# kkromberg/SpeechRecognition

Hardware: AMD Instinct MI355X
Metric: frames/sec scored+decoded (higher is better)
Workload: dtype f64

## Files before the change

speechrecognition_amd/csrc/gmm_prefilter.hip:

```cpp
#include <hip/hip_runtime.h>
#include <stdint.h>

#include <algorithm>
#include <cmath>
#include <vector>

#include "kernels.h"

#ifndef SR_P16_NB
#define SR_P16_NB 4
#endif

namespace srgpu {

typedef float v4f __attribute__((ext_vector_type(4)));
static constexpr int kPWaves = 4;
static constexpr int kGroupBlocks = 8;

typedef _Float16 f16x8 __attribute__((ext_vector_type(8)));

__device__ inline uint32_t pack_f16x2(_Float16 l, _Float16 h) {
  return (uint32_t)__builtin_bit_cast(uint16_t, l) | ((uint32_t)__builtin_bit_cast(uint16_t, h) << 16);
}

template <int KS32, int NB>
__global__ __launch_bounds__(kPWaves * 64, (NB <= 2 ? 3 : 2)) void gmm_prefilter16_kernel(GmmPrefilterArgs a) {
  constexpr int kBlockBytes = KS32 * 1024;
  constexpr int kStageBytes = kGroupBlocks * kBlockBytes;
  constexpr int kChunksPerStage = kStageBytes / 1024;
  constexpr int kDmaPerWave = kChunksPerStage / kPWaves;
  static_assert(kChunksPerStage % kPWaves == 0, "every wave issues the same number of LDS-DMA pieces per stage");
  constexpr int kTileFrames = kPWaves * NB * 16;
  constexpr size_t kTileBytes = (size_t)kTileFrames * (16 * KS32) * sizeof(float);
  constexpr size_t kLdsBytes = 2 * kStageBytes > kTileBytes ? 2 * kStageBytes : kTileBytes;
  __shared__ __attribute__((aligned(1024))) unsigned char lds[kLdsBytes];

  const int lane = threadIdx.x & 63, wave = threadIdx.x >> 6;
  const int g = lane >> 4, c = lane & 15;
  uint32_t x, y;
  {
    const uint32_t id = blockIdx.x;
    if ((a.ny & 7u) == 0) { const uint32_t j = id >> 3; y = (id & 7u) + 8u * (j / a.nx); x = j % a.nx; }
    else { y = id / a.nx; x = id % a.nx; }
  }
  const uint32_t g0 = a.split_begin[y], g1 = a.split_begin[y + 1];
  const uint64_t frame0 = (uint64_t)x * kTileFrames + (uint64_t)wave * (NB * 16);

  uint4 bf[NB][KS32];
  float bnorm[NB], dbnorm[NB];
  {
    float* fl = reinterpret_cast<float*>(lds);
    const uint64_t tile_first = (uint64_t)x * kTileFrames;
    const uint64_t tile_frames = (a.n_frames - tile_first < (uint64_t)kTileFrames) ? a.n_frames - tile_first : kTileFrames;
    const uint32_t n_floats = (uint32_t)tile_frames * a.dim;
    const float* src = a.feats + tile_first * a.dim;
    for (uint32_t i = threadIdx.x; i < n_floats; i += kPWaves * 64) fl[i] = src[i];
    __syncthreads();
#pragma unroll
    for (int nb = 0; nb < NB; nb++) {
      const uint32_t row = (uint32_t)wave * (NB * 16) + nb * 16 + c;
      const bool valid = row < tile_frames;
      const float* xr = fl + (valid ? row : 0u) * a.dim;
      float n2 = 0.0f, e2 = 0.0f;
#pragma unroll
      for (int ks = 0; ks < KS32; ks++) {
        _Float16 v[8];
#pragma unroll
        for (int j = 0; j < 8; j++) {
          const uint32_t k = 32u * ks + 8u * g + j, d = k >> 1;
          const float xf = (valid && d < a.dim) ? xr[d < a.dim ? d : 0u] : 0.0f;
          const float b = (k & 1u) ? xf : xf * xf;
          n2 += b * b;
          _Float16 h = (_Float16)b;
          const float bh = (float)h;
          const float e = (k & 1u) ? xf - bh : __builtin_fmaf(xf, xf, -bh);
          e2 += e * e;
          if (valid && k >= 2u * a.dim && k < 2u * a.dim + 3u) h = (_Float16)1.0f;
          v[j] = h;
        }
        bf[nb][ks] = make_uint4(pack_f16x2(v[0], v[1]), pack_f16x2(v[2], v[3]), pack_f16x2(v[4], v[5]), pack_f16x2(v[6], v[7]));
      }
      n2 += __shfl_xor(n2, 16);
      n2 += __shfl_xor(n2, 32);
      e2 += __shfl_xor(e2, 16);
      e2 += __shfl_xor(e2, 32);
      bnorm[nb] = sqrtf(n2) * 1.0001f;
      dbnorm[nb] = fminf(sqrtf(e2) * 1.0001f, kPfRes16 * bnorm[nb]);
    }
    __syncthreads();
  }

  const unsigned char* dma_src = a.apack + (uint64_t)g0 * kStageBytes + (uint64_t)wave * 1024 + lane * 16;
  auto issue_stage = [&](int buf) {
#pragma unroll
    for (int i = 0; i < kDmaPerWave; i++) {
      const int chunk = i * kPWaves + wave;
      unsigned char* dst = lds + buf * kStageBytes + chunk * 1024;
      __builtin_amdgcn_global_load_lds((const __attribute__((address_space(1))) void*)(dma_src + i * (kPWaves * 1024)),
                                       (__attribute__((address_space(3))) void*)dst, 16, 0, 0);
    }
    dma_src += kStageBytes;
  };
  auto frag = [&](int buf, int j, int ks) -> f16x8 {
    return __builtin_bit_cast(f16x8, *reinterpret_cast<const uint4*>(lds + buf * kStageBytes + j * kBlockBytes + ks * 1024 + lane * 16));
  };

  const uint32_t n_stages = g1 - g0;
  if (n_stages > 0) issue_stage(0);
  if (n_stages > 1) issue_stage(1);
  if (n_stages > 1) __builtin_amdgcn_s_waitcnt(0x0F70 | kDmaPerWave);
  else __builtin_amdgcn_s_waitcnt(0x0F70);
  __syncthreads();
  f16x8 a_c, a_n;
  if (n_stages > 0) a_c = frag(0, 0, 0);
  uint32_t* m_ptr = a.mask + (uint64_t)g0 * a.n_frames * 4u;
  uint32_t m_off[NB];
  bool m_ok[NB];
#pragma unroll
  for (int nb = 0; nb < NB; nb++) {
    const uint64_t f = frame0 + (uint64_t)nb * 16 + c;
    m_ok[nb] = f < a.n_frames;
    m_off[nb] = (uint32_t)f * 4u + (uint32_t)g;
  }
  for (uint32_t s = 0; s < n_stages; s++) {
    const uint32_t grp = g0 + s;
    const int buf = s & 1;
    v4f ap[NB][kGroupBlocks];
#pragma unroll
    for (int j = 0; j < kGroupBlocks; j++) {
      v4f acc[NB];
#pragma unroll
      for (int nb = 0; nb < NB; nb++) acc[nb] = (v4f){0.f, 0.f, 0.f, 0.f};
#pragma unroll
      for (int ks = 0; ks < KS32; ks++) {
        if (j == kGroupBlocks - 1 && ks == KS32 - 1) {
          if (s + 1 < n_stages) {
            __builtin_amdgcn_s_waitcnt(0x0070);
            __syncthreads();
            if (s + 2 < n_stages) issue_stage(buf);
            a_n = frag(buf ^ 1, 0, 0);
          }
        } else {
          a_n = frag(buf, (ks == KS32 - 1) ? j + 1 : j, (ks == KS32 - 1) ? 0 : ks + 1);
        }
        __builtin_amdgcn_sched_barrier(0);
#pragma unroll
        for (int nb = 0; nb < NB; nb++)
          acc[nb] = __builtin_amdgcn_mfma_f32_16x16x32_f16(a_c, __builtin_bit_cast(f16x8, bf[nb][ks]), acc[nb], 0, 0, 0);
        __builtin_amdgcn_sched_barrier(0);
        a_c = a_n;
      }
#pragma unroll
      for (int nb = 0; nb < NB; nb++) ap[nb][j] = acc[nb];
    }
    const float4 lim = reinterpret_cast<const float4*>(a.grp_lim)[4u * grp + g];
#pragma unroll
    for (int nb = 0; nb < NB; nb++) {
      float amin = __builtin_huge_valf();
#pragma unroll
      for (int j = 0; j < kGroupBlocks; j += 2)
        asm("v_min3_f32 %0, %0, %1, %2\n\tv_min3_f32 %0, %0, %3, %4\n\tv_min3_f32 %0, %0, %5, %6\n\tv_min3_f32 %0, %0, %7, %8"
            : "+v"(amin)
            : "v"(ap[nb][j][0]), "v"(ap[nb][j][1]), "v"(ap[nb][j][2]), "v"(ap[nb][j][3]), "v"(ap[nb][j + 1][0]),
              "v"(ap[nb][j + 1][1]), "v"(ap[nb][j + 1][2]), "v"(ap[nb][j + 1][3]));
      if (a.chunks >= 2) { const float o = __shfl_xor(amin, 16); asm("v_min_f32 %0, %0, %1" : "+v"(amin) : "v"(o)); }
      if (a.chunks >= 4) { const float o = __shfl_xor(amin, 32); asm("v_min_f32 %0, %0, %1" : "+v"(amin) : "v"(o)); }
      const float limit = amin + __builtin_fmaf(lim.y, dbnorm[nb], __builtin_fmaf(lim.x, bnorm[nb], lim.z));
      uint32_t mask = 0;
#pragma unroll
      for (int j = kGroupBlocks - 1; j >= 1; j -= 2)
        asm("v_cmp_ngt_f32 vcc, %2, %1\n\tv_addc_co_u32 %0, vcc, %0, %0, vcc\n\t"
            "v_cmp_ngt_f32 vcc, %3, %1\n\tv_addc_co_u32 %0, vcc, %0, %0, vcc\n\t"
            "v_cmp_ngt_f32 vcc, %4, %1\n\tv_addc_co_u32 %0, vcc, %0, %0, vcc\n\t"
            "v_cmp_ngt_f32 vcc, %5, %1\n\tv_addc_co_u32 %0, vcc, %0, %0, vcc\n\t"
            "v_cmp_ngt_f32 vcc, %6, %1\n\tv_addc_co_u32 %0, vcc, %0, %0, vcc\n\t"
            "v_cmp_ngt_f32 vcc, %7, %1\n\tv_addc_co_u32 %0, vcc, %0, %0, vcc\n\t"
            "v_cmp_ngt_f32 vcc, %8, %1\n\tv_addc_co_u32 %0, vcc, %0, %0, vcc\n\t"
            "v_cmp_ngt_f32 vcc, %9, %1\n\tv_addc_co_u32 %0, vcc, %0, %0, vcc"
            : "+v"(mask)
            : "v"(limit), "v"(ap[nb][j][3]), "v"(ap[nb][j][2]), "v"(ap[nb][j][1]), "v"(ap[nb][j][0]), "v"(ap[nb][j - 1][3]),
              "v"(ap[nb][j - 1][2]), "v"(ap[nb][j - 1][1]), "v"(ap[nb][j - 1][0])
            : "vcc");
      if (m_ok[nb]) m_ptr[m_off[nb]] = mask;
    }
    m_ptr += a.n_frames * 4u;
  }
}

#ifndef SR_PS_PIN
#define SR_PS_PIN 1
#endif
#if SR_PS_PIN
#define SR_PS_PIN_FETCH __builtin_amdgcn_sched_barrier(0)
#else
#define SR_PS_PIN_FETCH (void)0
#endif
static constexpr int kSNB = 2;
static constexpr int kSRangeFrames = 2048;

template <int KS32>
__global__ __launch_bounds__(kPWaves * 64) void gmm_prefilter_operands_kernel(const float* feats, uint64_t n_frames, uint32_t dim,
                                                                              uint64_t n_blocks, uint4* bfrag, float2* bnorm) {
  const int lane = threadIdx.x & 63, wave = threadIdx.x >> 6;
  const uint32_t g = lane >> 4, c = lane & 15;
  const uint64_t blk = (uint64_t)blockIdx.x * kPWaves + wave;
  if (blk >= n_blocks) return;
  const uint64_t f = blk * 16 + c;
  const bool valid = f < n_frames;
  const float* xr = feats + (valid ? f : 0u) * dim;
  float n2 = 0.0f, e2 = 0.0f;
#pragma unroll
  for (int ks = 0; ks < KS32; ks++) {
    _Float16 v[8];
#pragma unroll
    for (int j = 0; j < 8; j++) {
      const uint32_t k = 32u * ks + 8u * g + j, d = k >> 1;
      const float xf = (valid && d < dim) ? xr[d < dim ? d : 0u] : 0.0f;
      const float b = (k & 1u) ? xf : xf * xf;
      n2 += b * b;
      _Float16 h = (_Float16)b;
      const float bh = (float)h;
      const float e = (k & 1u) ? xf - bh : __builtin_fmaf(xf, xf, -bh);
      e2 += e * e;
      if (valid && k >= 2u * dim && k < 2u * dim + 3u) h = (_Float16)1.0f;
      v[j] = h;
    }
    bfrag[(blk * KS32 + ks) * 64 + lane] =
        make_uint4(pack_f16x2(v[0], v[1]), pack_f16x2(v[2], v[3]), pack_f16x2(v[4], v[5]), pack_f16x2(v[6], v[7]));
  }
  n2 += __shfl_xor(n2, 16);
  n2 += __shfl_xor(n2, 32);
  e2 += __shfl_xor(e2, 16);
  e2 += __shfl_xor(e2, 32);
  const float bn = sqrtf(n2) * 1.0001f;
  const float dbn = fminf(sqrtf(e2) * 1.0001f, kPfRes16 * bn);
  if (g == 0) bnorm[f] = make_float2(bn, dbn);
}

struct GmmStationaryPlan { uint32_t n_quads, n_ranges, range_frames, per_xcd; };

template <int KS32>
__global__ __launch_bounds__(kPWaves * 64, 2) void gmm_prefilter_stationary_kernel(GmmPrefilterArgs a, GmmStationaryPlan p) {
  constexpr int NB = kSNB;
  constexpr int kGroupBytes = kGroupBlocks * KS32 * 1024;
  const int lane = threadIdx.x & 63, wave = threadIdx.x >> 6;
  const int g = lane >> 4, c = lane & 15;
  const uint32_t item = (blockIdx.x & 7u) * p.per_xcd + (blockIdx.x >> 3);
  if ((blockIdx.x >> 3) >= p.per_xcd || item >= p.n_quads * p.n_ranges) return;
  const uint32_t grp = (item % p.n_quads) * kPWaves + wave;
  if (grp >= a.n_groups) return;
  const uint64_t f_begin = (uint64_t)(item / p.n_quads) * p.range_frames;
  if (f_begin >= a.n_frames) return;
  const uint64_t f_end = f_begin + p.range_frames < a.n_frames ? f_begin + p.range_frames : a.n_frames;
  const uint32_t n_steps = (uint32_t)((f_end - f_begin + 16 * NB - 1) / (16 * NB));

  f16x8 af[kGroupBlocks][KS32];
  {
    const uint4* src = reinterpret_cast<const uint4*>(a.apack + (uint64_t)grp * kGroupBytes) + lane;
#pragma unroll
    for (int j = 0; j < kGroupBlocks; j++)
#pragma unroll
      for (int ks = 0; ks < KS32; ks++) af[j][ks] = __builtin_bit_cast(f16x8, src[(j * KS32 + ks) * 64]);
  }
  const float4 lim = reinterpret_cast<const float4*>(a.grp_lim)[4u * grp + g];

  const uint4* b_src = a.bfrag + (f_begin / 16) * (KS32 * 64) + lane;
  const float2* n_src = a.bnorm + f_begin + c;
  uint32_t* m_ptr = a.mask + (uint64_t)grp * a.n_frames * 4u;
  uint4 bq[2][NB][KS32];
  float2 nq[2][NB];
  auto fetch = [&](int buf, uint32_t s) __attribute__((always_inline)) {
    const uint4* bs = b_src + (uint64_t)s * (NB * KS32 * 64);
#pragma unroll
    for (int nb = 0; nb < NB; nb++) {
#pragma unroll
      for (int ks = 0; ks < KS32; ks++) bq[buf][nb][ks] = bs[(nb * KS32 + ks) * 64];
      nq[buf][nb] = n_src[(uint64_t)s * (NB * 16) + nb * 16];
    }
  };
  auto step = [&](int buf, uint32_t s) __attribute__((always_inline)) {
    v4f ap[NB][kGroupBlocks];
#pragma unroll
    for (int nb = 0; nb < NB; nb++)
#pragma unroll
      for (int j = 0; j < kGroupBlocks; j++) ap[nb][j] = (v4f){0.f, 0.f, 0.f, 0.f};
#pragma unroll
    for (int ks = 0; ks < KS32; ks++)
#pragma unroll
      for (int j = 0; j < kGroupBlocks; j++)
#pragma unroll
        for (int nb = 0; nb < NB; nb++)
          ap[nb][j] = __builtin_amdgcn_mfma_f32_16x16x32_f16(af[j][ks], __builtin_bit_cast(f16x8, bq[buf][nb][ks]), ap[nb][j], 0, 0, 0);
    __builtin_amdgcn_sched_barrier(0);
    asm volatile("s_nop 7");
    __builtin_amdgcn_sched_barrier(0);
#pragma unroll
    for (int nb = 0; nb < NB; nb++) {
      float amin = __builtin_huge_valf();
#pragma unroll
      for (int j = 0; j < kGroupBlocks; j += 2)
        asm("v_min3_f32 %0, %0, %1, %2\n\tv_min3_f32 %0, %0, %3, %4\n\tv_min3_f32 %0, %0, %5, %6\n\tv_min3_f32 %0, %0, %7, %8"
            : "+v"(amin)
            : "v"(ap[nb][j][0]), "v"(ap[nb][j][1]), "v"(ap[nb][j][2]), "v"(ap[nb][j][3]), "v"(ap[nb][j + 1][0]),
              "v"(ap[nb][j + 1][1]), "v"(ap[nb][j + 1][2]), "v"(ap[nb][j + 1][3]));
      if (a.chunks >= 2) { const float o = __shfl_xor(amin, 16); asm("v_min_f32 %0, %0, %1" : "+v"(amin) : "v"(o)); }
      if (a.chunks >= 4) { const float o = __shfl_xor(amin, 32); asm("v_min_f32 %0, %0, %1" : "+v"(amin) : "v"(o)); }
      const float limit = amin + __builtin_fmaf(lim.y, nq[buf][nb].y, __builtin_fmaf(lim.x, nq[buf][nb].x, lim.z));
      uint32_t mask = 0;
#pragma unroll
      for (int j = kGroupBlocks - 1; j >= 1; j -= 2)
        asm("v_cmp_ngt_f32 vcc, %2, %1\n\tv_addc_co_u32 %0, vcc, %0, %0, vcc\n\t"
            "v_cmp_ngt_f32 vcc, %3, %1\n\tv_addc_co_u32 %0, vcc, %0, %0, vcc\n\t"
            "v_cmp_ngt_f32 vcc, %4, %1\n\tv_addc_co_u32 %0, vcc, %0, %0, vcc\n\t"
            "v_cmp_ngt_f32 vcc, %5, %1\n\tv_addc_co_u32 %0, vcc, %0, %0, vcc\n\t"
            "v_cmp_ngt_f32 vcc, %6, %1\n\tv_addc_co_u32 %0, vcc, %0, %0, vcc\n\t"
            "v_cmp_ngt_f32 vcc, %7, %1\n\tv_addc_co_u32 %0, vcc, %0, %0, vcc\n\t"
            "v_cmp_ngt_f32 vcc, %8, %1\n\tv_addc_co_u32 %0, vcc, %0, %0, vcc\n\t"
            "v_cmp_ngt_f32 vcc, %9, %1\n\tv_addc_co_u32 %0, vcc, %0, %0, vcc"
            : "+v"(mask)
            : "v"(limit), "v"(ap[nb][j][3]), "v"(ap[nb][j][2]), "v"(ap[nb][j][1]), "v"(ap[nb][j][0]), "v"(ap[nb][j - 1][3]),
              "v"(ap[nb][j - 1][2]), "v"(ap[nb][j - 1][1]), "v"(ap[nb][j - 1][0])
            : "vcc");
      const uint64_t f = f_begin + (uint64_t)s * (NB * 16) + nb * 16 + c;
      if (f < a.n_frames) m_ptr[(uint32_t)f * 4u + (uint32_t)g] = mask;
    }
  };
  fetch(0, 0);
  for (uint32_t s = 0; s < n_steps; s += 2) {
    fetch(1, s + 1 < n_steps ? s + 1 : n_steps - 1);
    SR_PS_PIN_FETCH;
    step(0, s);
    if (s + 1 >= n_steps) break;
    fetch(0, s + 2 < n_steps ? s + 2 : n_steps - 1);
    SR_PS_PIN_FETCH;
    step(1, s + 1);
  }
}

__global__ void fp16_denormal_probe_kernel(float* out) {
  const int lane = threadIdx.x;
  f16x8 a = {0, 0, 0, 0, 0, 0, 0, 0}, b = {0, 0, 0, 0, 0, 0, 0, 0};
  if (lane < 16) { a[0] = (_Float16)9.5367431640625e-7f; b[0] = (_Float16)1024.0f; }
  v4f acc = {0.f, 0.f, 0.f, 0.f};
  acc = __builtin_amdgcn_mfma_f32_16x16x32_f16(a, b, acc, 0, 0, 0);
  out[lane] = acc[0];
}

hipError_t probe_fp16_denormals(hipStream_t stream, bool* preserved) {
  float* d = nullptr;
  hipError_t e = hipMalloc(reinterpret_cast<void**>(&d), 64 * sizeof(float));
  if (e != hipSuccess) return e;
  hipLaunchKernelGGL(fp16_denormal_probe_kernel, dim3(1), dim3(64), 0, stream, d);
  float h[64];
  e = hipGetLastError();
  if (e == hipSuccess) e = hipStreamSynchronize(stream);
  if (e == hipSuccess) e = hipMemcpy(h, d, sizeof(h), hipMemcpyDeviceToHost);
  (void)hipFree(d);
  if (e != hipSuccess) return e;
  *preserved = true;
  for (int i = 0; i < 64; i++) *preserved = *preserved && h[i] == 9.765625e-4f;
  return hipSuccess;
}

template <int KS>
__global__ void fp16_accumulation_probe_kernel(const _Float16* A, const _Float16* B, float* out) {
  constexpr int K = 32 * KS;
  const int lane = threadIdx.x, r = lane & 15, q = lane >> 4;
  v4f acc = {0.f, 0.f, 0.f, 0.f};
#pragma unroll
  for (int ks = 0; ks < KS; ks++) {
    f16x8 a, b;
#pragma unroll
    for (int j = 0; j < 8; j++) {
      const int k = 32 * ks + 8 * q + j;
      a[j] = A[r * K + k];
      b[j] = B[k * 16 + r];
    }
    acc = __builtin_amdgcn_mfma_f32_16x16x32_f16(a, b, acc, 0, 0, 0);
  }
#pragma unroll
  for (int i = 0; i < 4; i++) out[(4 * q + i) * 16 + r] = acc[i];
}

hipError_t probe_fp16_accumulation(hipStream_t stream, int ks32, bool* ok, double* worst_ratio) {
  if (ks32 != 3 && ks32 != 4) return hipErrorInvalidValue;
  const int kCases = 8;
  const int K = 32 * ks32;
  const double allowed = ks32 == 3 ? 87.0 : 132.0;
  std::vector<_Float16> hA((size_t)kCases * 16 * K), hB((size_t)kCases * K * 16);
  uint64_t rng = 0x9E3779B97F4A7C15ull;
  auto next = [&]() { rng ^= rng << 13; rng ^= rng >> 7; rng ^= rng << 17; return rng; };
  for (int t = 0; t < kCases; t++) {
    _Float16* A = hA.data() + (size_t)t * 16 * K;
    _Float16* B = hB.data() + (size_t)t * K * 16;
    for (int k = 0; k < K; k++)
      for (int c = 0; c < 16; c++) B[k * 16 + c] = (_Float16)1.0f;
    for (int r = 0; r < 16; r++)
      for (int k = 0; k < K; k++) {
        float a = 0.f;
        const int fam = (t * 16 + r) & 3;
        if (fam == 0) a = k == (r * 5) % K ? 4096.0f : 0.75f;
        else if (fam == 1) a = k >= K - 2 ? 0.f : ((k & 1) ? -1.f : 1.f) * (1024.0f + (float)(((k >> 1) * 7 + r) % 64) * ((k & 1) ? 0.5f : 0.53125f));
        else if (fam == 2) a = 1.0009765625f;
        else { const uint64_t u = next(); a = ((u & 1) ? -1.f : 1.f) * (1.0f + (float)((u >> 8) & 1023) / 1024.0f) * (float)(1u << ((u >> 20) % 12)); }
        A[r * K + k] = (_Float16)a;
      }
    for (int k = 0; k < K; k++)
      for (int c = 0; c < 16; c++) {
        const uint64_t u = next();
        float b = 1.0f + (float)((u >> 5) % 1024) / 1024.0f;
        if ((c & 3) == 0) b = 1.0f;
        if ((c & 3) == 1) b = 1.0009765625f;
        B[k * 16 + c] = (_Float16)b;
      }
    for (int c = 0; c < 16; c++)
      for (int r = 0; r < 16; r++)
        if (((t * 16 + r) & 3) == 0) B[((r * 5) % K) * 16 + c] = (_Float16)2048.0f;
  }
  _Float16 *dA = nullptr, *dB = nullptr;
  float* dO = nullptr;
  hipError_t e;
  if ((e = hipMalloc(reinterpret_cast<void**>(&dA), hA.size() * 2)) != hipSuccess) return e;
  if ((e = hipMalloc(reinterpret_cast<void**>(&dB), hB.size() * 2)) != hipSuccess) { (void)hipFree(dA); return e; }
  if ((e = hipMalloc(reinterpret_cast<void**>(&dO), (size_t)kCases * 256 * 4)) != hipSuccess) { (void)hipFree(dA); (void)hipFree(dB); return e; }
  std::vector<float> got((size_t)kCases * 256);
  e = hipMemcpy(dA, hA.data(), hA.size() * 2, hipMemcpyHostToDevice);
  if (e == hipSuccess) e = hipMemcpy(dB, hB.data(), hB.size() * 2, hipMemcpyHostToDevice);
  for (int t = 0; t < kCases && e == hipSuccess; t++) {
    if (ks32 == 3) hipLaunchKernelGGL(fp16_accumulation_probe_kernel<3>, dim3(1), dim3(64), 0, stream, dA + (size_t)t * 16 * K, dB + (size_t)t * K * 16, dO + (size_t)t * 256);
    else hipLaunchKernelGGL(fp16_accumulation_probe_kernel<4>, dim3(1), dim3(64), 0, stream, dA + (size_t)t * 16 * K, dB + (size_t)t * K * 16, dO + (size_t)t * 256);
    e = hipGetLastError();
  }
  if (e == hipSuccess) e = hipStreamSynchronize(stream);
  if (e == hipSuccess) e = hipMemcpy(got.data(), dO, got.size() * 4, hipMemcpyDeviceToHost);
  (void)hipFree(dA); (void)hipFree(dB); (void)hipFree(dO);
  if (e != hipSuccess) return e;
  double worst = 0.0;
  bool fine = true;
  for (int t = 0; t < kCases; t++)
    for (int r = 0; r < 16; r++)
      for (int c = 0; c < 16; c++) {
        double exact = 0.0, mag = 0.0;
        for (int k = 0; k < K; k++) {
          const double p = (double)(float)hA[((size_t)t * 16 + r) * K + k] * (double)(float)hB[((size_t)t * K + k) * 16 + c];
          exact += p;
          mag += p < 0 ? -p : p;
        }
        const double err = std::fabs((double)got[(size_t)t * 256 + r * 16 + c] - exact);
        const double ratio = err / (mag * 5.9604644775390625e-8);
        if (!(ratio <= allowed)) fine = false;
        if (ratio > worst || ratio != ratio) worst = ratio;
      }
  *ok = fine;
  if (worst_ratio) *worst_ratio = worst;
  return hipSuccess;
}

static GmmStationaryPlan stationary_plan(uint32_t n_groups, uint64_t n_frames) {
  GmmStationaryPlan p{};
  p.n_quads = (n_groups + kPWaves - 1) / kPWaves;
  const uint64_t steps = (n_frames + 16 * kSNB - 1) / (16 * kSNB);
  const uint64_t r_max = std::max<uint64_t>(1, std::min<uint64_t>(steps, (n_frames + kSRangeFrames - 1) / kSRangeFrames));
  uint64_t best_r = 1;
  double best = -1.0;
  for (uint64_t r = 1; r <= r_max; r++) {
    const uint64_t wgs = (uint64_t)p.n_quads * r;
    const double fill = (double)wgs / (double)((wgs + 511) / 512 * 512);
    if (fill > best * (1.0 + 1e-9)) { best = fill; best_r = r; }
  }
  const uint64_t range_steps = (steps + best_r - 1) / best_r;
  p.range_frames = (uint32_t)(range_steps * 16 * kSNB);
  p.n_ranges = (uint32_t)((steps + range_steps - 1) / range_steps);
  p.per_xcd = (uint32_t)(((uint64_t)p.n_quads * p.n_ranges + 7) / 8);
  return p;
}

int gmm_prefilter_route(int ks32, int route) { return (route == kPfStationary && ks32 >= 1 && ks32 <= 3) ? kPfStationary : kPfStaged; }
int gmm_prefilter_stationary_range_frames() { return kSRangeFrames; }
void gmm_prefilter_operand_sizes(int ks32, uint64_t n_frames, size_t* n_frag, size_t* n_norm) {
  const uint64_t blocks = (n_frames + 16 * kSNB - 1) / (16 * kSNB) * kSNB;
  *n_frag = (size_t)blocks * ks32 * 64;
  *n_norm = (size_t)blocks * 16;
}

template <int KS32>
static hipError_t launch_stationary(const GmmPrefilterArgs& a, hipStream_t stream) {
  if (!a.bfrag || !a.bnorm || a.n_groups == 0) return hipErrorInvalidValue;
  size_t n_frag, n_norm;
  gmm_prefilter_operand_sizes(KS32, a.n_frames, &n_frag, &n_norm);
  const uint64_t blocks = n_norm / 16;
  hipLaunchKernelGGL((gmm_prefilter_operands_kernel<KS32>), dim3((unsigned)((blocks + kPWaves - 1) / kPWaves)), dim3(kPWaves * 64), 0, stream,
                     a.feats, a.n_frames, a.dim, blocks, a.bfrag, a.bnorm);
  hipError_t e = hipGetLastError();
  if (e != hipSuccess) return e;
  const GmmStationaryPlan p = stationary_plan(a.n_groups, a.n_frames);
  hipLaunchKernelGGL((gmm_prefilter_stationary_kernel<KS32>), dim3(8 * p.per_xcd), dim3(kPWaves * 64), 0, stream, a, p);
  return hipGetLastError();
}

hipError_t launch_gmm_prefilter(const GmmPrefilterArgs& a, int ks32, int route, hipStream_t stream) {
  if (a.n_frames >= (1ull << 30)) return hipErrorInvalidValue;
  if (a.n_frames == 0) return hipSuccess;
  if (gmm_prefilter_route(ks32, route) == kPfStationary) {
    switch (ks32) {
      case 1: return launch_stationary<1>(a, stream);
      case 2: return launch_stationary<2>(a, stream);
      default: return launch_stationary<3>(a, stream);
    }
  }
  const dim3 grid(a.nx * a.ny), block(kPWaves * 64);
  switch (ks32) {
    case 1: hipLaunchKernelGGL((gmm_prefilter16_kernel<1, SR_P16_NB>), grid, block, 0, stream, a); break;
    case 2: hipLaunchKernelGGL((gmm_prefilter16_kernel<2, SR_P16_NB>), grid, block, 0, stream, a); break;
    case 3: hipLaunchKernelGGL((gmm_prefilter16_kernel<3, SR_P16_NB>), grid, block, 0, stream, a); break;
    case 4: hipLaunchKernelGGL((gmm_prefilter16_kernel<4, SR_P16_NB>), grid, block, 0, stream, a); break;
    default: return hipErrorInvalidValue;
  }
  return hipGetLastError();
}
int gmm_prefilter_frames_per_tile() { return kPWaves * SR_P16_NB * 16; }

#pragma clang fp contract(off)

#ifndef SR_R_THREADS
#define SR_R_THREADS 768
#endif
#ifndef SR_R_BATCH
#define SR_R_BATCH 4
#endif
static constexpr int kRThreads = SR_R_THREADS;
static constexpr int kRThreadsWide = 512;
static constexpr int kRWaves = kRThreads / 64;
static constexpr int kRBatch = SR_R_BATCH;
#ifndef SR_R_BATCH_WIDE
#define SR_R_BATCH_WIDE 8
#endif
static constexpr int kRBatchWide = SR_R_BATCH_WIDE;
static constexpr uint32_t kRingEntries = 128;
static constexpr uint32_t kRingLists = 2 * 8 * kRingEntries;
static constexpr uint32_t kRingWave = 4 * kRingLists;
struct __attribute__((aligned(16))) RingEntry { uint32_t lf, mask; double score; };
struct __attribute__((packed, aligned(4))) RowPiece { float v[4]; };

template <int DT, int NS, int SPW, int CH, int NT = kRThreads, int VS = 1, bool DEFER = false>
__global__ __launch_bounds__(NT) void gmm_refine_kernel(GmmRefineArgs a) {
  static_assert(DT > 0 && (DT & 1), "padded dimension: odd");
  static_assert(!DEFER || CH > 1, "deferred lists: states of several chunks");
  constexpr int kRThreads = NT, kRWaves = NT / 64;
  static_assert(CH == 1 || CH == 2 || CH == 4, "chunks per state (half)");
  static_assert(VS == 1 || (VS == 2 && CH == 4), "two halves only of four-chunk states");
  static_assert(SPW % (CH * VS) == 0 && (CH == 1 || SPW % 4 == 0), "a state's chunks live in one workgroup");
  extern __shared__ __attribute__((aligned(1024))) unsigned char panel_raw[];
  const uint32_t D = (uint32_t)DT, tid = threadIdx.x;
  const int lane = tid & 63, wave = tid >> 6;
  const uint32_t s0 = blockIdx.x * SPW;
  const uint32_t ns = (s0 + SPW <= a.n_pstates) ? SPW : a.n_pstates - s0;
  const uint32_t state_bytes = (2u * D + 2u) * NS * 8u;
  const uint64_t f_begin = (uint64_t)blockIdx.y * a.frames_per_split;
  const uint64_t f_end = (f_begin + a.frames_per_split < a.n_frames) ? f_begin + a.frames_per_split : a.n_frames;

  {
    const uint32_t chunks = (ns * state_bytes + 1023u) >> 10;
    const unsigned char* src = reinterpret_cast<const unsigned char*>(a.rows) + (uint64_t)s0 * state_bytes + lane * 16;
    for (uint32_t ch = wave; ch < chunks; ch += kRWaves)
      __builtin_amdgcn_global_load_lds((const __attribute__((address_space(1))) void*)(src + (uint64_t)ch * 1024u),
                                       (__attribute__((address_space(3))) void*)(panel_raw + ch * 1024u), 16, 0, 0);
  }
  uint32_t nd[SPW];
#pragma unroll
  for (int j = 0; j < SPW; j++) nd[j] = (uint32_t)j < ns ? a.n_dens_ps[s0 + j] : 0u;
  __builtin_amdgcn_s_waitcnt(0x0F70);
  __syncthreads();
  if (f_begin >= f_end) return;

  uint32_t n_eval = 0;
  double x[DT];
  const __amdgpu_buffer_rsrc_t featsT_rsrc = __builtin_amdgcn_make_buffer_rsrc(
      const_cast<float*>(a.featsT), 0, (int)0xFFFFFFFFu, 0x00020000);
  const uint32_t ld4 = (uint32_t)a.n_frames_ld * 4u;
  auto load_x = [&](uint64_t f) __attribute__((always_inline)) {
    const uint32_t voff = (uint32_t)f * 4u;
#pragma unroll
    for (int k = 0; k < DT; k++)
      x[k] = (double)__builtin_bit_cast(float, __builtin_amdgcn_raw_buffer_load_b32(featsT_rsrc, voff, (uint32_t)k * ld4, 0));
  };
  auto load_x_row = [&](uint64_t f) __attribute__((always_inline)) {
    const float* xr = a.feats + f * (uint64_t)DT;
#pragma unroll
    for (int q = 0; q < DT / 4; q++) {
      const RowPiece t = reinterpret_cast<const RowPiece*>(xr)[q];
#pragma unroll
      for (int i = 0; i < 4; i++) x[4 * q + i] = (double)t.v[i];
    }
#pragma unroll
    for (int k = DT - DT % 4; k < DT; k++) x[k] = (double)xr[k];
  };
  auto evaluate = [&](const unsigned char* col0) __attribute__((always_inline)) -> double {
    const volatile __attribute__((address_space(3))) double* col =
        (const volatile __attribute__((address_space(3))) double*)col0;
    double l0 = 0.0, l1 = 0.0, dist, score;
    {
      constexpr int RB = NT == kRThreadsWide ? kRBatchWide : kRBatch;
      constexpr int NB_ = (DT + 1 + RB - 1) / RB;
      double pm[2][RB], pv[2][RB];
#pragma unroll
      for (int i = 0; i < RB; i++)
        if (i <= DT) { pm[0][i] = col[(2 * i) * NS]; pv[0][i] = col[(2 * i + 1) * NS]; }
#pragma unroll
      for (int b = 0; b < NB_; b++) {
        const int cur = b & 1;
        __builtin_amdgcn_sched_barrier(0);
#pragma unroll
        for (int i = 0; i < RB; i++) {
          const int k = (b + 1) * RB + i;
          if (k <= DT) { pm[cur ^ 1][i] = col[(2 * k) * NS]; pv[cur ^ 1][i] = col[(2 * k + 1) * NS]; }
        }
        __builtin_amdgcn_sched_barrier(0);
#pragma unroll
        for (int i = 0; i < RB; i++) {
          const int k = b * RB + i;
          if (k < (int)(DT - (DT & 1))) {
            double u = x[k] - pm[cur][i];
            u = u * u;
            u = u * pv[cur][i];
            if (k & 1) l1 = l1 + u; else l0 = l0 + u;
          } else if (k == DT - 1) {
            dist = l0 + l1;
            const double t = x[k] - pm[cur][i];
            dist += t * t * pv[cur][i];
          } else if (k == DT) {
            if (!(DT & 1)) dist = l0 + l1;
            score = pm[cur][i] + dist / 2;
            score -= pv[cur][i];
          }
        }
        asm volatile("" : "+v"(l0), "+v"(l1));
      }
    }
    return score;
// ... 571 lines not shown
```

Baseline: 13.97 million.

## Software-pipeline MFMA accumulation with previous tile's min/compare/mask epilogue

Restructures the stationary prefilter kernel so each half-step issues the MFMAs for one 16-frame block while the min-reduction, limit computation, threshold comparisons and mask store for the previous block are interleaved between them via sched_barriers. This is meant to hide the MFMA result latency and the serial VALU epilogue (previously separated by an s_nop and run after all MFMAs) behind matrix work. It adds a one-block lag with a drain iteration and more live accumulator registers, which risks register pressure and occupancy at two waves per SIMD.

```diff
diff --git a/speechrecognition_amd/csrc/gmm_prefilter.hip b/speechrecognition_amd/csrc/gmm_prefilter.hip
--- a/speechrecognition_amd/csrc/gmm_prefilter.hip
+++ b/speechrecognition_amd/csrc/gmm_prefilter.hip
@@ -3,6 +3,7 @@
 
 #include <algorithm>
 #include <cmath>
+#include <type_traits>
 #include <vector>
 
 #include "kernels.h"
@@ -195,6 +196,9 @@
 #else
 #define SR_PS_PIN_FETCH (void)0
 #endif
+#ifndef SR_PS_PIPE
+#define SR_PS_PIPE 1
+#endif
 static constexpr int kSNB = 2;
 static constexpr int kSRangeFrames = 2048;
 
@@ -238,6 +242,14 @@
 }
 
 struct GmmStationaryPlan { uint32_t n_quads, n_ranges, range_frames, per_xcd; };
+
+template <int I, int E, class F>
+__device__ __forceinline__ void static_for(F&& f) {
+  if constexpr (I < E) {
+    f(std::integral_constant<int, I>{});
+    static_for<I + 1, E>(f);
+  }
+}
 
 template <int KS32>
 __global__ __launch_bounds__(kPWaves * 64, 2) void gmm_prefilter_stationary_kernel(GmmPrefilterArgs a, GmmStationaryPlan p) {
@@ -278,6 +290,72 @@
       nq[buf][nb] = n_src[(uint64_t)s * (NB * 16) + nb * 16];
     }
   };
+#if SR_PS_PIPE
+  constexpr int kPieces = 23;
+  v4f ap[NB][kGroupBlocks];
+  float lfr[NB];
+#pragma unroll
+  for (int j = 0; j < kGroupBlocks; j++) ap[1][j] = (v4f){0.f, 0.f, 0.f, 0.f};
+  lfr[1] = 0.f;
+  auto half = [&](auto bufc, auto nbc, uint64_t fp, bool store_on) __attribute__((always_inline)) {
+    constexpr int buf = decltype(bufc)::value, nb = decltype(nbc)::value, pb = nb ^ 1;
+    constexpr int G = kGroupBlocks * KS32;
+    float amin = __builtin_huge_valf(), limit = 0.f;
+    uint32_t mask = 0;
+    static_for<0, G>([&](auto mc) __attribute__((always_inline)) {
+      constexpr int m = decltype(mc)::value, ks = m / kGroupBlocks, j = m % kGroupBlocks;
+      if constexpr (ks == 0)
+        ap[nb][j] = __builtin_amdgcn_mfma_f32_16x16x32_f16(af[j][ks], __builtin_bit_cast(f16x8, bq[buf][nb][ks]), (v4f){0.f, 0.f, 0.f, 0.f}, 0, 0, 0);
+      else
+        ap[nb][j] = __builtin_amdgcn_mfma_f32_16x16x32_f16(af[j][ks], __builtin_bit_cast(f16x8, bq[buf][nb][ks]), ap[nb][j], 0, 0, 0);
+      __builtin_amdgcn_sched_barrier(0);
+      static_for<0, kPieces>([&](auto pc) __attribute__((always_inline)) {
+        constexpr int p = decltype(pc)::value;
+        if constexpr (p * G / kPieces == m) {
+          if constexpr (p < 4) {
+            asm("v_min3_f32 %0, %0, %1, %2\n\tv_min3_f32 %0, %0, %3, %4\n\tv_min3_f32 %0, %0, %5, %6\n\tv_min3_f32 %0, %0, %7, %8"
+                : "+v"(amin)
+                : "v"(ap[pb][2 * p][0]), "v"(ap[pb][2 * p][1]), "v"(ap[pb][2 * p][2]), "v"(ap[pb][2 * p][3]), "v"(ap[pb][2 * p + 1][0]),
+                  "v"(ap[pb][2 * p + 1][1]), "v"(ap[pb][2 * p + 1][2]), "v"(ap[pb][2 * p + 1][3]));
+          } else if constexpr (p == 4) {
+            if (a.chunks >= 2) { const float o = __shfl_xor(amin, 16); asm("v_min_f32 %0, %0, %1" : "+v"(amin) : "v"(o)); }
+            if (a.chunks >= 4) { const float o = __shfl_xor(amin, 32); asm("v_min_f32 %0, %0, %1" : "+v"(amin) : "v"(o)); }
+            limit = amin + lfr[pb];
+          } else if constexpr (p < 21) {
+            constexpr int e = 4 * kGroupBlocks - 1 - 2 * (p - 5);
+            asm("v_cmp_ngt_f32 vcc, %2, %1\n\tv_addc_co_u32 %0, vcc, %0, %0, vcc\n\t"
+                "v_cmp_ngt_f32 vcc, %3, %1\n\tv_addc_co_u32 %0, vcc, %0, %0, vcc"
+                : "+v"(mask)
+                : "v"(limit), "v"(ap[pb][e >> 2][e & 3]), "v"(ap[pb][(e - 1) >> 2][(e - 1) & 3])
+                : "vcc");
+          } else if constexpr (p == 21) {
+            if (store_on && fp < a.n_frames) m_ptr[(uint32_t)fp * 4u + (uint32_t)g] = mask;
+          } else {
+            lfr[nb] = __builtin_fmaf(lim.y, nq[buf][nb].y, __builtin_fmaf(lim.x, nq[buf][nb].x, lim.z));
+            asm volatile("" : "+v"(lfr[nb]));
+          }
+        }
+      });
+      __builtin_amdgcn_sched_barrier(0);
+    });
+  };
+  const std::integral_constant<int, 0> c0;
+  const std::integral_constant<int, 1> c1;
+  const uint64_t f0 = f_begin + (uint64_t)c;
+  fetch(0, 0);
+  for (uint32_t s = 0;; s += 2) {
+    fetch(1, s + 1 < n_steps ? s + 1 : n_steps - 1);
+    SR_PS_PIN_FETCH;
+    half(c0, c0, f0 + (uint64_t)s * (NB * 16) - 16, s > 0);
+    if (s >= n_steps) break;
+    half(c0, c1, f0 + (uint64_t)s * (NB * 16), true);
+    fetch(0, s + 2 < n_steps ? s + 2 : n_steps - 1);
+    SR_PS_PIN_FETCH;
+    half(c1, c0, f0 + (uint64_t)s * (NB * 16) + 16, true);
+    if (s + 1 >= n_steps) break;
+    half(c1, c1, f0 + (uint64_t)s * (NB * 16) + 32, true);
+  }
+#else
   auto step = [&](int buf, uint32_t s) __attribute__((always_inline)) {
     v4f ap[NB][kGroupBlocks];
 #pragma unroll
@@ -335,6 +413,7 @@
     SR_PS_PIN_FETCH;
     step(1, s + 1);
   }
+#endif
 }
 
 __global__ void fp16_denormal_probe_kernel(float* out) {
```

Result: no change. 13.99 million (median of 2 runs) (+0.1%).
